# SFR-Vision/6d-pose-estimation

Measured on NVIDIA B200. Metric: ADD-S pose evals/sec (2k-pt mesh), higher is better.
Workload: dtype f32

## Files before the change

6d-pose-estimation_b200/csrc/p6d_adds_pruned.cu:

```cuda
#include <algorithm>
#include <memory>
#include <vector>

#include "p6d_common.cuh"

namespace p6d {

constexpr int PR_BLOCK = 32;
constexpr int PR_SUB = 8;

struct PrunedSlot {
    int64_t offset;
    int32_t nb;
    int32_t floats;
};
__host__ __device__ inline int pr_floats(int nb) {
    const int np = PR_BLOCK * nb, nbp = (nb + 3) / 4 * 4;
    return 3 * np + 3 * nbp + 12 * nb + np / 2;
}

struct PrunedTable {
    float* d_sorted = nullptr;
    PrunedSlot* d_slots = nullptr;
    std::vector<PrunedSlot> h_slots;
    int max_nb = 0;
    int max_count = 0;
};

static void kd_split(const float* xyz, std::vector<int>& idx, int lo, int hi) {
    if (hi - lo <= PR_SUB) return;
    const int unit = hi - lo > PR_BLOCK ? PR_BLOCK : PR_SUB;
    float mn[3] = {1e30f, 1e30f, 1e30f}, mx[3] = {-1e30f, -1e30f, -1e30f};
    for (int i = lo; i < hi; ++i)
        for (int c = 0; c < 3; ++c) {
            const float v = xyz[3 * idx[i] + c];
            if (v < mn[c]) mn[c] = v;
            if (v > mx[c]) mx[c] = v;
        }
    int axis = 0;
    for (int c = 1; c < 3; ++c)
        if (mx[c] - mn[c] > mx[axis] - mn[axis]) axis = c;
    const int blocks = (hi - lo + unit - 1) / unit;
    const int mid = lo + (blocks + 1) / 2 * unit;
    auto key = [&](int i) { const float v = xyz[3 * i + axis]; return v == v ? v : 3.0e38f; };
    std::nth_element(idx.begin() + lo, idx.begin() + mid, idx.begin() + hi, [&](int a, int b) {
        const float va = key(a), vb = key(b);
        return va < vb || (va == vb && a < b);
    });
    kd_split(xyz, idx, lo, mid);
    kd_split(xyz, idx, mid, hi);
}

static PrunedTable* build_blocks(const p6d_mesh_table* t, const float* xyz, const int32_t* offsets) {
    std::unique_ptr<PrunedTable> pt(new PrunedTable());
    pt->h_slots.resize(t->n_slots);
    size_t total = 0;
    for (int s = 0; s < t->n_slots; ++s) {
        const int n = t->h_slots[s].count;
        PrunedSlot& ps = pt->h_slots[s];
        ps.nb = (n + PR_BLOCK - 1) / PR_BLOCK;
        ps.floats = pr_floats(ps.nb);
        ps.offset = static_cast<int64_t>(total);
        total += static_cast<size_t>(ps.floats);
        pt->max_nb = std::max(pt->max_nb, ps.nb);
        pt->max_count = std::max(pt->max_count, n);
    }
    std::vector<float> buf(total > 0 ? total : 4, 0.0f);
    for (int s = 0; s < t->n_slots; ++s) {
        const int n = t->h_slots[s].count;
        if (n == 0) continue;
        const PrunedSlot& ps = pt->h_slots[s];
        const float* src = xyz + 3 * static_cast<size_t>(offsets[s]);
        std::vector<int> idx(n);
        for (int i = 0; i < n; ++i) idx[i] = i;
        kd_split(src, idx, 0, n);
        const int np = PR_BLOCK * ps.nb, nbp = (ps.nb + 3) / 4 * 4;
        float* x = buf.data() + ps.offset;
        float* cen = x + 3 * np;
        float* sub = cen + 3 * nbp;
        const int ns = 4 * ps.nb;
        uint16_t* perm = reinterpret_cast<uint16_t*>(sub + 3 * ns);
        for (int b = 0; b < ps.nb; ++b) {
            double c[3] = {0.0, 0.0, 0.0};
            const int cnt = std::min(PR_BLOCK, n - PR_BLOCK * b);
            for (int l = 0; l < PR_BLOCK; ++l) {
                const int p = PR_BLOCK * b + l;
                const int i = idx[l < cnt ? p : PR_BLOCK * b];
                for (int k = 0; k < 3; ++k) x[k * np + p] = src[3 * i + k];
                perm[p] = l < cnt ? static_cast<uint16_t>(i) : 0xffffu;
                if (l < cnt)
                    for (int k = 0; k < 3; ++k) c[k] += src[3 * i + k];
            }
            for (int k = 0; k < 3; ++k) cen[k * nbp + b] = static_cast<float>(c[k] / cnt);
            for (int q = 0; q < PR_BLOCK / PR_SUB; ++q) {
                double sc[3] = {0.0, 0.0, 0.0};
                const int first = PR_BLOCK * b + PR_SUB * q;
                const int scnt = std::max(0, std::min(PR_SUB, n - first));
                for (int l = 0; l < scnt; ++l)
                    for (int k = 0; k < 3; ++k) sc[k] += x[k * np + first + l];
                for (int k = 0; k < 3; ++k)
                    sub[k * ns + 4 * b + q] = scnt > 0 ? static_cast<float>(sc[k] / scnt) : x[k * np + PR_BLOCK * b];
            }
        }
    }
    if (cudaMalloc(&pt->d_sorted, buf.size() * sizeof(float)) != cudaSuccess ||
        cudaMalloc(&pt->d_slots, t->n_slots * sizeof(PrunedSlot)) != cudaSuccess ||
        cudaMemcpy(pt->d_sorted, buf.data(), buf.size() * sizeof(float), cudaMemcpyHostToDevice) != cudaSuccess ||
        cudaMemcpy(pt->d_slots, pt->h_slots.data(), t->n_slots * sizeof(PrunedSlot), cudaMemcpyHostToDevice) !=
            cudaSuccess) {
        cudaGetLastError();
        if (pt->d_sorted) cudaFree(pt->d_sorted);
        if (pt->d_slots) cudaFree(pt->d_slots);
        return nullptr;
    }
    return pt.release();
}

PrunedTable* build_pruned(const p6d_mesh_table* t, const float* xyz, const int32_t* offsets) {
    if (t->max_count > 65534) return nullptr;
    try {
        return build_blocks(t, xyz, offsets);
    } catch (...) {
        return nullptr;
    }
}

void free_pruned(PrunedTable* pt) {
    if (!pt) return;
    cudaFree(pt->d_sorted);
    cudaFree(pt->d_slots);
    delete pt;
}

struct PrunedArgs {
    const float* sorted;
    const PrunedSlot* pslots;
};

__host__ __device__ inline size_t pr_smem_floats(int nb, int nmax) {
    const int np = PR_BLOCK * nb;
    return static_cast<size_t>(pr_floats(nb)) + 3 * np + 3 * np + 2 * static_cast<size_t>((nmax + 3) / 4 * 4) + 4 * nb + 16 * nb;
}

__device__ __forceinline__ float eval_block(const float4* __restrict__ q, float px, float py, float pz, float m) {
    float m2 = __int_as_float(0x7f800000);
#pragma unroll
    for (int k = 0; k < PR_BLOCK / 4; ++k) {
        const float4 X = q[3 * k], Y = q[3 * k + 1], Z = q[3 * k + 2];
        pair_tile(px, py, pz, make_float2(X.x, X.y), make_float2(Y.x, Y.y), make_float2(Z.x, Z.y), m);
        pair_tile(px, py, pz, make_float2(X.z, X.w), make_float2(Y.z, Y.w), make_float2(Z.z, Z.w), m2);
    }
    return min_nan(m, m2);
}

__device__ __forceinline__ float eval_sub(const float4* __restrict__ q, float px, float py, float pz, float m) {
    float m2 = __int_as_float(0x7f800000);
#pragma unroll
    for (int k = 0; k < PR_SUB / 4; ++k) {
        const float4 X = q[3 * k], Y = q[3 * k + 1], Z = q[3 * k + 2];
        pair_tile(px, py, pz, make_float2(X.x, X.y), make_float2(Y.x, Y.y), make_float2(Z.x, Z.y), m);
        pair_tile(px, py, pz, make_float2(X.z, X.w), make_float2(Y.z, Y.w), make_float2(Z.z, Z.w), m2);
    }
    return min_nan(m, m2);
}

__device__ __forceinline__ float eval_two(const float4* __restrict__ q0, const float4* __restrict__ q1, float px, float py,
                                          float pz, float m) {
    const float a = eval_sub(q0, px, py, pz, m);
    const float b = eval_sub(q1, px, py, pz, __int_as_float(0x7f800000));
    return min_nan(a, b);
}

template <int T, int MINB>
__global__ void __launch_bounds__(T, MINB) adds_pruned_kernel(EvalArgs a, PrunedArgs pa, int nb_max, int nmax) {
    constexpr int PR_WARPS = T / 32;
    extern __shared__ __align__(128) unsigned char smem_raw[];
    const int np_max = PR_BLOCK * nb_max;
    float* s_sorted = reinterpret_cast<float*>(smem_raw);
    float* s_gt = s_sorted + pr_floats(nb_max);
    float* s_pred = s_gt + 3 * np_max;
    float* s_dadd = s_pred + 3 * np_max;
    float* s_dadds = s_dadd + (nmax + 3) / 4 * 4;
    float4* s_cp = reinterpret_cast<float4*>(s_dadds + (nmax + 3) / 4 * 4);
    float4* s_cg = s_cp + nb_max;
    __shared__ uint64_t s_bar;
    __shared__ float s_pose[14];
    __shared__ float s_mean[2];
    __shared__ long long s_oid;
    __shared__ int s_next;
    __shared__ int s_blk[2];

    const unsigned full = 0xffffffffu;
    const int tid = threadIdx.x, lane = tid & 31, warp = tid >> 5;
    if (tid == 0) {
        mbar_init(&s_bar, 1);
        fence_mbar_init();
        s_blk[0] = PR_WARPS;
        s_blk[1] = PR_WARPS;
    }
    int par = 0;
    long long staged_oid = -1;
    uint32_t phase = 0;
    if (tid == 0) s_next = atomicAdd(a.work_counter, 1);
    __syncthreads();

    for (;;) {
        const int64_t it = s_next;
        if (it >= a.B) break;
        const int64_t b = a.order ? a.order[it] : it;
        load_pose(a, b, tid, s_pose, &s_oid);
        __syncthreads();
        if (tid == 64) s_next = atomicAdd(a.work_counter, 1);
        const long long oid = s_oid;
        if (!slot_known(oid, a.n_slots, a.slots)) {
            if (tid == 0) write_skipped(a, b, true);
            __syncthreads();
            continue;
        }
        const SlotInfo s = a.slots[oid];
        const PrunedSlot ps = pa.pslots[oid];
        const int n = s.count, nb = ps.nb, np = PR_BLOCK * nb, nbp = (nb + 3) / 4 * 4;
        if (oid != staged_oid) {
            stage_mesh(s_sorted, pa.sorted + ps.offset, ps.floats, &s_bar, phase, tid);
            phase ^= 1;
            staged_oid = oid;
        }
        const float* mx = s_sorted;
        const float* my = mx + np;
        const float* mz = my + np;
        const float* cen = mz + np;
        const float* sub = cen + 3 * nbp;
        const int ns = 4 * nb;
        const uint16_t* perm = reinterpret_cast<const uint16_t*>(sub + 3 * ns);
        const int mode = s.xform_mode;

        {
            float Rp[9], Rg[9], tp[3], tg[3];
            quat_to_mat(s_pose, Rp);
            quat_to_mat(s_pose + 4, Rg);
#pragma unroll
            for (int k = 0; k < 3; ++k) {
                tp[k] = s_pose[8 + k];
                tg[k] = s_pose[11 + k];
            }
            for (int blk = warp; blk < nb; blk += PR_WARPS) {
                const int p = PR_BLOCK * blk + lane;
                const unsigned orig = perm[p];
                const bool valid = orig != 0xffffu;
                const float x = mx[p], y = my[p], z = mz[p];
                float px, py, pz, qx, qy, qz;
                xform_point(mode, x, y, z, Rp, tp, px, py, pz);
                xform_point(mode, x, y, z, Rg, tg, qx, qy, qz);
                s_pred[p] = px;
                s_pred[np + p] = py;
                s_pred[2 * np + p] = pz;
                float* gq = s_gt + (p >> 2) * 12 + (p & 3);
                gq[0] = valid ? qx : GT_SENTINEL;
                gq[4] = valid ? qy : GT_SENTINEL;
                gq[8] = valid ? qz : GT_SENTINEL;
                if (valid) s_dadd[orig] = __fsqrt_rn(sq3(__fsub_rn(px, qx), __fsub_rn(py, qy), __fsub_rn(pz, qz)));
                const float cx = cen[blk], cy = cen[nbp + blk], cz = cen[2 * nbp + blk];
                const int sb = 4 * blk + (lane >> 3);
                const float sx = sub[sb], sy = sub[ns + sb], sz = sub[2 * ns + sb];
                float cpx, cpy, cpz, cgx, cgy, cgz;
                xform_point(XF_FMA_CHAIN, cx, cy, cz, Rp, tp, cpx, cpy, cpz);
                xform_point(XF_FMA_CHAIN, sx, sy, sz, Rg, tg, cgx, cgy, cgz);
                const float dp = sqrtf(sq3(px - cpx, py - cpy, pz - cpz));
                const float dg = sqrtf(sq3(qx - cgx, qy - cgy, qz - cgz));
                const unsigned rp = __reduce_max_sync(full, valid ? __float_as_uint(dp) : 0u);
                unsigned rg = valid ? __float_as_uint(dg) : 0u;
                rg = max(rg, __shfl_xor_sync(full, rg, 1));
                rg = max(rg, __shfl_xor_sync(full, rg, 2));
                rg = max(rg, __shfl_xor_sync(full, rg, 4));
                if (lane == 0) s_cp[blk] = make_float4(cpx, cpy, cpz, __uint_as_float(rp) * 1.00001f);
                if ((lane & 7) == 0) s_cg[sb] = make_float4(cgx, cgy, cgz, __uint_as_float(rg) * 1.00001f);
            }
        }
        __syncthreads();

        {
            const float4* gq4 = reinterpret_cast<const float4*>(s_gt);
            int A = warp;
            while (A < nb) {
                const int p = PR_BLOCK * A + lane;
                const unsigned orig = perm[p];
                const bool valid = orig != 0xffffu;
                const float px = s_pred[p], py = s_pred[np + p], pz = s_pred[2 * np + p];
                float m = eval_block(gq4 + 24 * A, px, py, pz, __int_as_float(0x7f800000));
                const float4 cA = s_cp[A];
                for (int c0 = 0; c0 < ns; c0 += 32) {
                    const float mmax = __uint_as_float(__reduce_max_sync(full, valid ? __float_as_uint(m) : 0u));
                    const float th = sqrtf(mmax) * 1.0001f + cA.w;
                    const int Bq = c0 + lane;
                    bool cand = false;
                    if (Bq < ns && (Bq >> 2) != A) {
                        const float4 cB = s_cg[Bq];
                        const float dx = cA.x - cB.x, dy = cA.y - cB.y, dz = cA.z - cB.z;
                        const float d2 = dx * dx + dy * dy + dz * dz;
                        const float rhs = th + cB.w;
                        const bool skip = d2 * 0.9999f >= rhs * rhs && d2 < 3.0e38f;
                        cand = !skip;
                    }
                    unsigned todo = __ballot_sync(full, cand);
                    while (todo) {
                        const int b0 = __ffs(todo) - 1;
                        todo &= todo - 1;
                        if (todo) {
                            const int b1 = __ffs(todo) - 1;
                            todo &= todo - 1;
                            m = eval_two(gq4 + 6 * (c0 + b0), gq4 + 6 * (c0 + b1), px, py, pz, m);
                        } else {
                            m = eval_sub(gq4 + 6 * (c0 + b0), px, py, pz, m);
                        }
                    }
                }
                if (valid) s_dadds[orig] = __fsqrt_rn(m);
                int nxt = 0;
                if (lane == 0) nxt = atomicAdd(&s_blk[par], 1);
                A = __shfl_sync(full, nxt, 0);
            }
        }
        __syncthreads();
        if (tid == 0) s_blk[par] = PR_WARPS;
        par ^= 1;

        if (tid < 64) {
            ordered_means(s_dadd, s_dadds, n, tid, lane, true, s_mean, [](const float* p) { return *p; });
            if (tid == 0) write_pose(a, b, oid, s, s_mean[0], s_mean[1], true);
        }
    }
}

static size_t pruned_smem_bytes(const p6d_mesh_table* t) {
    const int nb = t->pruned->max_nb > 0 ? t->pruned->max_nb : 1;
    return sizeof(float) * pr_smem_floats(nb, t->max_count);
}

bool pruned_fits(const p6d_mesh_table* t, int limit) {
    return pruned_smem_bytes(t) + 1024 <= static_cast<size_t>(limit);
}

int launch_eval_pruned(const p6d_mesh_table* table, const EvalArgs& args, cudaStream_t st) {
    const PrunedTable* ptab = table->pruned;
    if (!ptab) {
        set_error("p6d_add_eval_pruned: this table has no block structure (a mesh with more than 65,534 points, or out of "
                  "memory at creation)");
        return P6D_ETOOBIG;
    }
    int limit = 0;
    int rc = max_optin_smem(table->device, &limit);
    if (rc) return rc;
    if (!pruned_fits(table, limit)) {
        set_error("largest mesh has %d points; the pruned ADD-S kernel keeps both clouds and the sorted mesh in "
                  "shared memory and accepts at most %d points on this device (p6d_add_eval takes larger meshes)",
                  table->max_count, (limit - 1024) / 4 / 12 / 32 * 32);
        return P6D_ETOOBIG;
    }
    const int nb = ptab->max_nb > 0 ? ptab->max_nb : 1;
    const size_t smem = pruned_smem_bytes(table);
    EvalArgs a = args;
    if ((rc = claim_counter(table, st, &a.work_counter))) return rc;
    struct Shape { const void* fn; int threads, minb; };
    const Shape shapes[] = {{(const void*)adds_pruned_kernel<128, 8>, 128, 8}, {(const void*)adds_pruned_kernel<256, 4>, 256, 4},
                            {(const void*)adds_pruned_kernel<256, 3>, 256, 3}, {(const void*)adds_pruned_kernel<256, 2>, 256, 2}};
    const Shape* pick = &shapes[3];
    int per_sm = 0;
    for (const Shape& sh : shapes) {
        if (sh.threads == 128 && nb > 16) continue;
        if ((rc = ctas_per_sm(sh.fn, sh.threads, table->device, smem, &per_sm))) return rc;
        if (per_sm >= sh.minb || &sh == &shapes[3]) {
            pick = &sh;
            break;
        }
    }
    int64_t grid = static_cast<int64_t>(table->sm_count) * per_sm;
    if (grid > a.B) grid = a.B;
    PrunedArgs pa{ptab->d_sorted, ptab->d_slots};
    int nb_arg = nb, nmax_arg = table->max_count;
    void* kargs[] = {&a, &pa, &nb_arg, &nmax_arg};
    P6D_CUDA(cudaLaunchKernel(pick->fn, dim3(static_cast<unsigned>(grid)), dim3(pick->threads), kargs, smem, st));
    P6D_CUDA(cudaGetLastError());
    return P6D_OK;
}

}
```

Measured before the change: 1.387 million.

## Add lean pruned ADD-S variant that reads mesh from global memory

Splits the pruned ADD-S kernel into staged and lean variants selected at launch. The lean variant drops the shared-memory copy of the sorted mesh and the predicted cloud. It reads mesh data via __ldg and recomputes predicted points from a shared transform during the search phase. This shrinks shared memory per CTA so more CTAs fit per SM, at the cost of extra global loads and repeated transforms. The staged variant is used only when it does not reduce occupancy.

New measurement: 1.387 million (median of 6 runs). About the same (+0.0%).

```diff
diff --git a/6d-pose-estimation_b200/csrc/p6d_adds_pruned.cu b/6d-pose-estimation_b200/csrc/p6d_adds_pruned.cu
--- a/6d-pose-estimation_b200/csrc/p6d_adds_pruned.cu
+++ b/6d-pose-estimation_b200/csrc/p6d_adds_pruned.cu
@@ -137,10 +137,13 @@
     const PrunedSlot* pslots;
 };
 
-__host__ __device__ inline size_t pr_smem_floats(int nb, int nmax) {
+__host__ __device__ inline size_t pr_smem_floats(int nb, int nmax, bool staged) {
     const int np = PR_BLOCK * nb;
-    return static_cast<size_t>(pr_floats(nb)) + 3 * np + 3 * np + 2 * static_cast<size_t>((nmax + 3) / 4 * 4) + 4 * nb + 16 * nb;
-}
+    return 3 * static_cast<size_t>(np) + 2 * static_cast<size_t>((nmax + 3) / 4 * 4) + 4 * nb + 16 * nb +
+           (staged ? static_cast<size_t>(pr_floats(nb)) + 3 * np : 0);
+}
+
+constexpr int PR_MAX_BLOCKS = 143;
 
 __device__ __forceinline__ float eval_block(const float4* __restrict__ q, float px, float py, float pz, float m) {
     float m2 = __int_as_float(0x7f800000);
@@ -171,24 +174,26 @@
     return min_nan(a, b);
 }
 
-template <int T, int MINB>
-__global__ void __launch_bounds__(T, MINB) adds_pruned_kernel(EvalArgs a, PrunedArgs pa, int nb_max, int nmax) {
+template <int T, bool STAGED>
+__device__ __forceinline__ void pruned_poses(const EvalArgs& a, const PrunedArgs& pa, int nb_max, int nmax) {
     constexpr int PR_WARPS = T / 32;
     extern __shared__ __align__(128) unsigned char smem_raw[];
     const int np_max = PR_BLOCK * nb_max;
-    float* s_sorted = reinterpret_cast<float*>(smem_raw);
-    float* s_gt = s_sorted + pr_floats(nb_max);
-    float* s_pred = s_gt + 3 * np_max;
-    float* s_dadd = s_pred + 3 * np_max;
+    float* s_gt = reinterpret_cast<float*>(smem_raw);
+    float* s_dadd = s_gt + 3 * np_max;
     float* s_dadds = s_dadd + (nmax + 3) / 4 * 4;
     float4* s_cp = reinterpret_cast<float4*>(s_dadds + (nmax + 3) / 4 * 4);
     float4* s_cg = s_cp + nb_max;
+    float* s_sorted = reinterpret_cast<float*>(s_cg + 4 * nb_max);
+    float* s_pred = s_sorted + pr_floats(nb_max);
     __shared__ uint64_t s_bar;
     __shared__ float s_pose[14];
+    __shared__ float s_xf[12];
     __shared__ float s_mean[2];
     __shared__ long long s_oid;
     __shared__ int s_next;
     __shared__ int s_blk[2];
+    __shared__ long long s_b;
 
     const unsigned full = 0xffffffffu;
     const int tid = threadIdx.x, lane = tid & 31, warp = tid >> 5;
@@ -208,6 +213,7 @@
         const int64_t it = s_next;
         if (it >= a.B) break;
         const int64_t b = a.order ? a.order[it] : it;
+        if (tid == 0) s_b = b;
         load_pose(a, b, tid, s_pose, &s_oid);
         __syncthreads();
         if (tid == 64) s_next = atomicAdd(a.work_counter, 1);
@@ -220,18 +226,20 @@
         const SlotInfo s = a.slots[oid];
         const PrunedSlot ps = pa.pslots[oid];
         const int n = s.count, nb = ps.nb, np = PR_BLOCK * nb, nbp = (nb + 3) / 4 * 4;
-        if (oid != staged_oid) {
-            stage_mesh(s_sorted, pa.sorted + ps.offset, ps.floats, &s_bar, phase, tid);
+        const float* tab = pa.sorted + ps.offset;
+        if (STAGED && oid != staged_oid) {
+            stage_mesh(s_sorted, tab, ps.floats, &s_bar, phase, tid);
             phase ^= 1;
             staged_oid = oid;
         }
-        const float* mx = s_sorted;
+        const float* mx = STAGED ? s_sorted : tab;
         const float* my = mx + np;
         const float* mz = my + np;
         const float* cen = mz + np;
         const float* sub = cen + 3 * nbp;
         const int ns = 4 * nb;
         const uint16_t* perm = reinterpret_cast<const uint16_t*>(sub + 3 * ns);
+        auto ld = [](const auto* q) { return STAGED ? *q : __ldg(q); };
         const int mode = s.xform_mode;
 
         {
@@ -243,25 +251,33 @@
                 tp[k] = s_pose[8 + k];
                 tg[k] = s_pose[11 + k];
             }
+            if (!STAGED && tid == 0) {
+#pragma unroll
+                for (int k = 0; k < 9; ++k) s_xf[k] = Rp[k];
+#pragma unroll
+                for (int k = 0; k < 3; ++k) s_xf[9 + k] = tp[k];
+            }
             for (int blk = warp; blk < nb; blk += PR_WARPS) {
                 const int p = PR_BLOCK * blk + lane;
-                const unsigned orig = perm[p];
+                const unsigned orig = ld(perm + p);
                 const bool valid = orig != 0xffffu;
-                const float x = mx[p], y = my[p], z = mz[p];
+                const float x = ld(mx + p), y = ld(my + p), z = ld(mz + p);
                 float px, py, pz, qx, qy, qz;
                 xform_point(mode, x, y, z, Rp, tp, px, py, pz);
                 xform_point(mode, x, y, z, Rg, tg, qx, qy, qz);
-                s_pred[p] = px;
-                s_pred[np + p] = py;
-                s_pred[2 * np + p] = pz;
+                if (STAGED) {
+                    s_pred[p] = px;
+                    s_pred[np + p] = py;
+                    s_pred[2 * np + p] = pz;
+                }
                 float* gq = s_gt + (p >> 2) * 12 + (p & 3);
                 gq[0] = valid ? qx : GT_SENTINEL;
                 gq[4] = valid ? qy : GT_SENTINEL;
                 gq[8] = valid ? qz : GT_SENTINEL;
                 if (valid) s_dadd[orig] = __fsqrt_rn(sq3(__fsub_rn(px, qx), __fsub_rn(py, qy), __fsub_rn(pz, qz)));
-                const float cx = cen[blk], cy = cen[nbp + blk], cz = cen[2 * nbp + blk];
+                const float cx = ld(cen + blk), cy = ld(cen + nbp + blk), cz = ld(cen + 2 * nbp + blk);
                 const int sb = 4 * blk + (lane >> 3);
-                const float sx = sub[sb], sy = sub[ns + sb], sz = sub[2 * ns + sb];
+                const float sx = ld(sub + sb), sy = ld(sub + ns + sb), sz = ld(sub + 2 * ns + sb);
                 float cpx, cpy, cpz, cgx, cgy, cgz;
                 xform_point(XF_FMA_CHAIN, cx, cy, cz, Rp, tp, cpx, cpy, cpz);
                 xform_point(XF_FMA_CHAIN, sx, sy, sz, Rg, tg, cgx, cgy, cgz);
@@ -283,9 +299,16 @@
             int A = warp;
             while (A < nb) {
                 const int p = PR_BLOCK * A + lane;
-                const unsigned orig = perm[p];
+                const unsigned orig = ld(perm + p);
                 const bool valid = orig != 0xffffu;
-                const float px = s_pred[p], py = s_pred[np + p], pz = s_pred[2 * np + p];
+                float px, py, pz;
+                if (STAGED) {
+                    px = s_pred[p];
+                    py = s_pred[np + p];
+                    pz = s_pred[2 * np + p];
+                } else {
+                    xform_point(mode, ld(mx + p), ld(my + p), ld(mz + p), s_xf, s_xf + 9, px, py, pz);
+                }
                 float m = eval_block(gq4 + 24 * A, px, py, pz, __int_as_float(0x7f800000));
                 const float4 cA = s_cp[A];
                 for (int c0 = 0; c0 < ns; c0 += 32) {
@@ -326,18 +349,31 @@
 
         if (tid < 64) {
             ordered_means(s_dadd, s_dadds, n, tid, lane, true, s_mean, [](const float* p) { return *p; });
-            if (tid == 0) write_pose(a, b, oid, s, s_mean[0], s_mean[1], true);
-        }
-    }
-}
-
-static size_t pruned_smem_bytes(const p6d_mesh_table* t) {
+            if (tid == 0) write_pose(a, s_b, oid, s, s_mean[0], s_mean[1], true);
+        }
+    }
+}
+
+template <int T, int MINB>
+__global__ void __launch_bounds__(T, MINB) adds_pruned_kernel(EvalArgs a, PrunedArgs pa, int nb_max, int nmax,
+                                                              int staged) {
+    if (staged) pruned_poses<T, true>(a, pa, nb_max, nmax);
+    else pruned_poses<T, false>(a, pa, nb_max, nmax);
+}
+
+static size_t pruned_smem_bytes(const p6d_mesh_table* t, bool staged) {
     const int nb = t->pruned->max_nb > 0 ? t->pruned->max_nb : 1;
-    return sizeof(float) * pr_smem_floats(nb, t->max_count);
+    return sizeof(float) * pr_smem_floats(nb, t->max_count, staged);
 }
 
 bool pruned_fits(const p6d_mesh_table* t, int limit) {
-    return pruned_smem_bytes(t) + 1024 <= static_cast<size_t>(limit);
+    return t->pruned->max_nb <= PR_MAX_BLOCKS && pruned_smem_bytes(t, false) + 1024 <= static_cast<size_t>(limit);
+}
+
+static int pruned_max_points(int limit) {
+    int nb = PR_MAX_BLOCKS;
+    while (nb > 1 && sizeof(float) * pr_smem_floats(nb, PR_BLOCK * nb, false) + 1024 > static_cast<size_t>(limit)) --nb;
+    return PR_BLOCK * nb;
 }
 
 int launch_eval_pruned(const p6d_mesh_table* table, const EvalArgs& args, cudaStream_t st) {
@@ -351,13 +387,13 @@
     int rc = max_optin_smem(table->device, &limit);
     if (rc) return rc;
     if (!pruned_fits(table, limit)) {
-        set_error("largest mesh has %d points; the pruned ADD-S kernel keeps both clouds and the sorted mesh in "
+        set_error("largest mesh has %d points; the pruned ADD-S kernel keeps the gt cloud and two distance rows in "
                   "shared memory and accepts at most %d points on this device (p6d_add_eval takes larger meshes)",
-                  table->max_count, (limit - 1024) / 4 / 12 / 32 * 32);
+                  table->max_count, pruned_max_points(limit));
         return P6D_ETOOBIG;
     }
     const int nb = ptab->max_nb > 0 ? ptab->max_nb : 1;
-    const size_t smem = pruned_smem_bytes(table);
+    const size_t lean = pruned_smem_bytes(table, false);
     EvalArgs a = args;
     if ((rc = claim_counter(table, st, &a.work_counter))) return rc;
     struct Shape { const void* fn; int threads, minb; };
@@ -367,17 +403,25 @@
     int per_sm = 0;
     for (const Shape& sh : shapes) {
         if (sh.threads == 128 && nb > 16) continue;
-        if ((rc = ctas_per_sm(sh.fn, sh.threads, table->device, smem, &per_sm))) return rc;
+        if ((rc = ctas_per_sm(sh.fn, sh.threads, table->device, lean, &per_sm))) return rc;
         if (per_sm >= sh.minb || &sh == &shapes[3]) {
             pick = &sh;
             break;
         }
     }
+    const size_t staged_bytes = pruned_smem_bytes(table, true);
+    int staged = 0;
+    if (staged_bytes + 1024 <= static_cast<size_t>(limit)) {
+        int per_sm_staged = 0;
+        if ((rc = ctas_per_sm(pick->fn, pick->threads, table->device, staged_bytes, &per_sm_staged))) return rc;
+        staged = per_sm_staged >= per_sm;
+    }
+    const size_t smem = staged ? staged_bytes : lean;
     int64_t grid = static_cast<int64_t>(table->sm_count) * per_sm;
     if (grid > a.B) grid = a.B;
     PrunedArgs pa{ptab->d_sorted, ptab->d_slots};
     int nb_arg = nb, nmax_arg = table->max_count;
-    void* kargs[] = {&a, &pa, &nb_arg, &nmax_arg};
+    void* kargs[] = {&a, &pa, &nb_arg, &nmax_arg, &staged};
     P6D_CUDA(cudaLaunchKernel(pick->fn, dim3(static_cast<unsigned>(grid)), dim3(pick->threads), kargs, smem, st));
     P6D_CUDA(cudaGetLastError());
     return P6D_OK;
```
